# xXJSONDeruloXx/linux-fg

Hardware: AMD Instinct MI355X
Metric: interpolated frames/s, 1080p->4K RGBA8 (higher is better)
Workload: dtype f32 arithmetic on u8 RGBA (u8 in, u8 out; int8 motion vectors); 1 GPU; 1080p->2160p scale+motion(8,16)+interpolate; order=one call per stage, semantics=reference, frames_in_flight=3, content=translated (the motion stage's best case but `static`; see content_sweep), parallelism=one frame pair per GPU x1, gpu_max_hw_queues=4

## Files before the change

### linux-fg_amd/csrc/motion_strip.hip

```cpp
#include "lfg_motion_common.hpp"

#include <algorithm>
#include <vector>

namespace lfg {

constexpr int kStripPix = 64 - (kB - 1);
constexpr int kStripThreads = 1024, kStripWaves = kStripThreads / 64;
constexpr int kStripWinLane = 64 + 2 * kR;
constexpr int kStripWarm = 4;
constexpr int kStripSync = 16;
constexpr int kStripListCap = 6;
constexpr uint32_t kKeyMask = 0xFFFFF800u;
constexpr uint32_t kNearD = 3u * 2048u + 2047u;
constexpr int kStripSlots = 64 * kStripCols;

typedef const __attribute__((address_space(3))) uint32_t *strip_lds_u32;

__device__ __forceinline__ float strip_shl1(float v) {
    return __builtin_bit_cast(float, __builtin_amdgcn_mov_dpp(__builtin_bit_cast(int, v), 0x130 , 0xF, 0xF, true));
}
__device__ __forceinline__ uint32_t strip_absdiff(uint32_t a, uint32_t b) {
    uint32_t d;
    asm("v_sad_u32 %0, %1, %2, 0" : "=v"(d) : "v"(a), "v"(b));
    return d;
}
__device__ __forceinline__ void strip_record(uint32_t *cnt, uint32_t *list, uint32_t key, uint32_t floor) {
    const uint32_t at = atomicAdd(cnt, 1u) & 0x7FFFFFFFu;
    if (at < (uint32_t)kStripListCap) { list[at] = key; return; }
    for (int k = 0; k < kStripListCap; ++k) {
        const uint32_t e = list[k];
        if (key > e && key - e > kNearD) return;
    }
    for (int k = 0; k < kStripListCap; ++k) {
        const uint32_t e = list[k];
        if (e > floor && e - floor > kNearD && atomicCAS(&list[k], e, key) == e) return;
    }
    atomicOr(cnt, 0x80000000u);
}
__device__ __forceinline__ uint32_t strip_and_or(uint32_t a, uint32_t m, uint32_t r) {
    uint32_t d;
    asm("v_and_or_b32 %0, %1, %2, %3" : "=v"(d) : "v"(a), "v"(m), "s"(r));
    return d;
}
__device__ __forceinline__ float strip_sum8_lanes(float v) {
    const float t2 = v + strip_shl1(v);
    const float t4 = t2 + strip_shl1(strip_shl1(t2));
    const float t8 = t4 + strip_shl1(strip_shl1(strip_shl1(strip_shl1(t4))));
    return t8;
}

struct StripArgs {
    const uint8_t *prev, *curr;
    int prevPitch, currPitch, W, H;
    int8_t *mv; int mvPitch;
    const uint32_t *order32, *rank2scan;
    uint32_t *colBand, *rowBand;
    uint32_t *tileFlags, *flagged; int flagTilesX;
    int chunksTall, chunksWide;
};

template <bool kTall, int kOut, int kEdge, bool kRankIsScan>
__device__ __forceinline__ void strip_item(const StripArgs &a, const int L0, const int I0, const uint32_t bit, uint32_t *sWin, uint32_t *sGmin, uint32_t *sCnt, uint32_t *sList,
                                           uint16_t *sFinal, uint16_t *sHard, float (*sDist)[kB * kB], const uint16_t *sScan, uint32_t &sHardN) {
    constexpr int kIn = kOut + kB - 1;
    constexpr int kWinIn = kIn + 2 * kR;
    constexpr int kP = kWinIn | 1;
    static_assert(kOut <= kStripCols, "the LDS arrays are laid out for kStripCols pixels across the edge at most");
    const int tid = threadIdx.x, lane = tid & 63;
    const int wave = __builtin_amdgcn_readfirstlane(tid >> 6);
    const int W = a.W, H = a.H;
    const int laneSize = kTall ? H : W;
    const int wl0 = L0 - kB / 2 - kR, wi0 = I0 - kB / 2 - kR;

    constexpr int jLo = kEdge == 0 ? kB / 2 : 0, jHi = kEdge == 1 ? kIn - (kB / 2 - 1) : kIn;
    auto inImage = [](int j) constexpr { return j >= jLo && j < jHi; };
    uint32_t c[kIn], cc[kIn];
    const int gl = L0 - kB / 2 + lane;
    const bool laneIn = gl >= 0 && gl < laneSize;
    const int edgeItem = __builtin_amdgcn_readfirstlane((int)(L0 - kB / 2 < 0 || L0 - kB / 2 + 63 >= laneSize));
    {
#pragma unroll
        for (int j = jLo; j < jHi; ++j) {
            const int gi = I0 - kB / 2 + j;
            const int x = kTall ? gi : gl, y = kTall ? gl : gi;
            c[j] = *reinterpret_cast<const uint32_t *>(a.curr + (size_t)clampi(y, 0, H - 1) * (size_t)a.currPitch + (size_t)clampi(x, 0, W - 1) * 4u);
        }
    }
    for (int e = tid; e < kStripWinLane * kWinIn; e += kStripThreads) {
        const int u = kTall ? e / kWinIn : e % kStripWinLane, v = kTall ? e % kWinIn : e / kStripWinLane;
        const int x = kTall ? wi0 + v : wl0 + u, y = kTall ? wl0 + u : wi0 + v;
        const uint32_t t = *reinterpret_cast<const uint32_t *>(a.prev + (size_t)clampi(y, 0, H - 1) * (size_t)a.prevPitch + (size_t)clampi(x, 0, W - 1) * 4u);
        sWin[u * kP + v] = (x >= 0 && x < W && y >= 0 && y < H) ? t : 0u;
    }
    for (int e = tid; e < kStripSlots; e += kStripThreads) { sGmin[e] = 0xFFFFFFFFu; sCnt[e] = 0u; }
    if (tid == 0) sHardN = 0u;
#pragma unroll
    for (int j = jLo; j < jHi; ++j) {
        cc[j] = __builtin_amdgcn_udot4(c[j], c[j], 0x4B000000u, false);
        asm volatile("" : "+v"(cc[j]));
    }
    __syncthreads();

    const bool laneOk = lane < kStripPix && L0 + lane < laneSize;
    uint32_t mn[kOut];
#pragma unroll
    for (int i = 0; i < kOut; ++i) mn[i] = 0xFFFFFFFFu;
    const strip_lds_u32 winLane = (strip_lds_u32)sWin + lane * kP;
    auto leaves = [&](int px, int py, uint32_t rank) {
        const uint32_t sc = kRankIsScan ? rank : (uint32_t)sScan[min(rank, (uint32_t)kCand - 1u)];
        const int dyi = (int)((sc * 1986u) >> 16), dxi = (int)sc - 33 * dyi;
        return block_leaves_prev(px, py, dxi - kR, dyi - kR, W, H);
    };
    auto inPlateau = [&](int i, uint32_t sc) {
        const int dyi = (int)((sc * 1986u) >> 16), dxi = (int)sc - 33 * dyi, dI = (kTall ? dxi : dyi) - kR;
        const int q = I0 + i;
        return q + kB / 2 - 1 + dI < 0 || q - kB / 2 + dI >= (kTall ? W : H);
    };
    if (wave == 0) {
#pragma unroll
        for (int i = 0; i < kOut; ++i) {
            uint32_t first = (uint32_t)kCand;
            for (int r0 = 0; r0 < kCand && first == (uint32_t)kCand; r0 += 64) {
                const int r = r0 + lane;
                const unsigned long long hit = __ballot(r < kCand && inPlateau(i, kRankIsScan ? (uint32_t)r : (uint32_t)sScan[min(r, kCand - 1)]));
                if (hit != 0ull) first = (uint32_t)(r0 + __builtin_ctzll(hit));
            }
            if (lane == 0) sHard[i] = (uint16_t)first;
        }
    }
    __syncthreads();
    uint32_t rep[kOut];
#pragma unroll
    for (int i = 0; i < kOut; ++i) rep[i] = (uint32_t)__builtin_amdgcn_readfirstlane((int)sHard[i]);
    __syncthreads();
    auto adopt = [&](int i, uint32_t g) {
        if (mn[i] != g && mn[i] - g <= kNearD && !(mn[i] < 2048u && g < 2048u) && (mn[i] & 0x7FFu) % (uint32_t)kStripWaves == (uint32_t)wave) {
            const int px = kTall ? I0 + i : L0 + lane, py = kTall ? L0 + lane : I0 + i;
            const bool plateau = (mn[i] >> 11) == (g >> 11) && leaves(px, py, mn[i] & 0x7FFu) && leaves(px, py, g & 0x7FFu);
            if (!plateau) strip_record(sCnt + lane * kOut + i, sList + (lane * kOut + i) * kStripListCap, mn[i], g);
        }
        mn[i] = g;
    };

    const int lanePlus2 = ((lane + 2) & 63) * 4, lanePlus4 = ((lane + 4) & 63) * 4;
    const int nMine = (kCand - wave + kStripWaves - 1) / kStripWaves;
    for (int t = 0; t < nMine + kStripWarm; ++t) {
        if (t == kStripWarm) {
            if (laneOk) {
#pragma unroll
                for (int i = 0; i < kOut; ++i) atomicMin(&sGmin[lane * kOut + i], mn[i]);
            }
            __syncthreads();
            if (laneOk) {
#pragma unroll
                for (int i = 0; i < kOut; ++i) mn[i] = sGmin[lane * kOut + i];
            }
        }
        else if (t > kStripWarm && ((t - kStripWarm) & (kStripSync - 1)) == 0) {
            if (laneOk) {
#pragma unroll
                for (int i = 0; i < kOut; ++i) atomicMin(&sGmin[lane * kOut + i], mn[i]);
#pragma unroll
                for (int i = 0; i < kOut; ++i) adopt(i, sGmin[lane * kOut + i]);
            }
        }
        const bool recording = t >= kStripWarm;
        const int r = wave + kStripWaves * (t < nMine ? t : t - nMine);
        const uint32_t sc = kRankIsScan ? (uint32_t)r : (uint32_t)sScan[r];
        const uint32_t dyi = (sc * 1986u) >> 16, dxi = sc - 33u * dyi;
        const uint32_t off = (kTall ? dyi : dxi) * (uint32_t)kP + (kTall ? dxi : dyi);
        const strip_lds_u32 w = winLane + off;
        uint32_t p[kIn];
#pragma unroll
        for (int j = jLo; j < jHi; ++j) p[j] = w[j];
        float d[kIn];
#pragma unroll
        for (int j = jLo; j < jHi; ++j) {
            const float f1 = __builtin_bit_cast(float, __builtin_amdgcn_udot4(p[j], p[j], cc[j], false));
            const float f2 = __builtin_bit_cast(float, __builtin_amdgcn_udot4(c[j], p[j], 0x4B800000u, false));
            d[j] = __builtin_amdgcn_sqrtf((f1 - f2) + 8388608.0f);
        }
        auto sum2 = [](float x, bool xIn, float y, bool yIn) { return xIn && yIn ? x + y : xIn ? x : yIn ? y : 0.0f; };
        auto in2 = [&](int j) constexpr { return inImage(j) || inImage(j + 1); };
        auto in4 = [&](int j) constexpr { return in2(j) || in2(j + 2); };
        float a2[kIn - 1], a4[kIn - 3], h8[kOut];
#pragma unroll
        for (int j = 0; j < kIn - 1; ++j) a2[j] = sum2(inImage(j) ? d[j] : 0.0f, inImage(j), inImage(j + 1) ? d[j + 1] : 0.0f, inImage(j + 1));
#pragma unroll
        for (int j = 0; j < kIn - 3; ++j) a4[j] = sum2(a2[j], in2(j), a2[j + 2], in2(j + 2));
#pragma unroll
        for (int i = 0; i < kOut; ++i) h8[i] = sum2(a4[i], in4(i), a4[i + 4], in4(i + 4));
        if (edgeItem) {
            asm volatile("; lanes outside the image (strip)");
#pragma unroll
            for (int i = 0; i < kOut; ++i) h8[i] = laneIn ? h8[i] : 0.0f;
        }
        float t2[kOut], t4[kOut], sum[kOut];
#pragma unroll
        for (int i = 0; i < kOut; ++i) t2[i] = h8[i] + strip_shl1(h8[i]);
#pragma unroll
        for (int i = 0; i < kOut; ++i) t4[i] = __builtin_bit_cast(float, __builtin_amdgcn_ds_bpermute(lanePlus2, __builtin_bit_cast(int, t2[i])));
#pragma unroll
        for (int i = 0; i < kOut; ++i) t4[i] = t2[i] + t4[i];
#pragma unroll
        for (int i = 0; i < kOut; ++i) sum[i] = __builtin_bit_cast(float, __builtin_amdgcn_ds_bpermute(lanePlus4, __builtin_bit_cast(int, t4[i])));
        uint32_t key[kOut], nearMin = 0xFFFFFFFFu;
#pragma unroll
        for (int i = 0; i < kOut; ++i) {
            const float s = t4[i] + sum[i];
            key[i] = strip_and_or(__builtin_bit_cast(uint32_t, s), kKeyMask, (uint32_t)r) | ((inPlateau(i, sc) && (uint32_t)r != rep[i]) ? 0xFFFFFFFFu : 0u);
            nearMin = min(nearMin, strip_absdiff(key[i], mn[i]));
        }
        nearMin = laneOk ? nearMin : 0xFFFFFFFFu;
        if (recording && __builtin_amdgcn_readfirstlane((int)(__ballot(nearMin <= kNearD) != 0ull))) {
            asm volatile("; near event (strip)");
#pragma unroll
            for (int i = 0; i < kOut; ++i) {
                const bool near = laneOk && strip_absdiff(key[i], mn[i]) <= kNearD;
                if (__builtin_amdgcn_readfirstlane((int)(__ballot(near) != 0ull))) {
                    if (near) {
                        const int px = kTall ? I0 + i : L0 + lane, py = kTall ? L0 + lane : I0 + i;
                        const uint32_t holder = mn[i];
                        bool skip = (key[i] < 2048u && holder < 2048u) || key[i] == holder;
                        if (!skip && (key[i] >> 11) == (holder >> 11)) skip = leaves(px, py, (uint32_t)r) && leaves(px, py, holder & 0x7FFu);
                        if (key[i] < holder && (holder & 0x7FFu) % (uint32_t)kStripWaves != (uint32_t)wave) skip = true;
                        if (!skip) strip_record(sCnt + lane * kOut + i, sList + (lane * kOut + i) * kStripListCap, max(key[i], holder), min(key[i], holder));
                    }
                }
            }
        }
#pragma unroll
        for (int i = 0; i < kOut; ++i) mn[i] = min(mn[i], key[i]);
    }

    if (laneOk) {
#pragma unroll
        for (int i = 0; i < kOut; ++i) atomicMin(&sGmin[lane * kOut + i], mn[i]);
    }
    __syncthreads();
    if (laneOk) {
#pragma unroll
        for (int i = 0; i < kOut; ++i) adopt(i, sGmin[lane * kOut + i]);
    }
    __syncthreads();
    for (int e = tid; e < kStripSlots; e += kStripThreads) {
        const int l = e / kOut, i = e - l * kOut;
        if (l >= kStripPix || L0 + l >= laneSize) continue;
        const uint32_t g = sGmin[e], n = sCnt[e];
        sFinal[e] = (uint16_t)(g & 0x7FFu);
        if (g < 2048u || n == 0u) continue;
        uint32_t live = 0u;
        for (uint32_t k = 0; k < min(n & 0x7FFFFFFFu, (uint32_t)kStripListCap); ++k) {
            const uint32_t key = sList[e * kStripListCap + k];
            live += (key >= g && key - g <= kNearD && key != g) ? 1u : 0u;
        }
        if ((n >> 31) != 0u) {
            const int px = kTall ? I0 + i : L0 + l, py = kTall ? L0 + l : I0 + i;
            if (atomicExch(&a.tileFlags[(py / kTH) * a.flagTilesX + px / kTW], 1u) == 0u) {
                const uint32_t slot = atomicAdd(a.flagged, 1u);
                if (slot < (uint32_t)kShareBelow) a.flagged[1 + slot] = (uint32_t)((py / kTH) * a.flagTilesX + px / kTW);
            }
            continue;
        }
        if (live == 0u) continue;
        sHard[atomicAdd(&sHardN, 1u)] = (uint16_t)e;
    }
    __syncthreads();
    const uint32_t hardN = sHardN;
    for (uint32_t hI = (uint32_t)wave; hI < hardN; hI += (uint32_t)kStripWaves) {
        const int e = (int)sHard[hI];
        const int l = e / kOut, i = e - l * kOut;
        const int qx = kTall ? I0 + i : L0 + l, qy = kTall ? L0 + l : I0 + i;
        const uint32_t g = sGmin[e];
        const uint32_t n = min(sCnt[e] & 0x7FFFFFFFu, (uint32_t)kStripListCap);
        uint32_t mine = 0xFFFFFFFFu;
        if (lane == 0) mine = g;
        else if ((uint32_t)lane <= n) { const uint32_t k = sList[e * kStripListCap + lane - 1]; mine = (k >= g && k - g <= kNearD) ? k : 0xFFFFFFFFu; }
        const int cx = qx - kB / 2 + (lane & 7), cy = qy - kB / 2 + (lane >> 3);
        const bool posIn = cx >= 0 && cx < W && cy >= 0 && cy < H;
        const uint32_t ctex = posIn ? *reinterpret_cast<const uint32_t *>(a.curr + (size_t)cy * (size_t)a.currPitch + (size_t)cx * 4u) : 0u;
        const float cf[4] = {unorm8_to_float(byte0(ctex)), unorm8_to_float(byte1(ctex)), unorm8_to_float(byte2(ctex)), unorm8_to_float(byte3(ctex))};
        float bestV = __builtin_inff();
        uint32_t bestR = 0xFFFFFFFFu, done = 0xFFFFFFFFu;
        unsigned long long todo = __ballot(mine != 0xFFFFFFFFu);
        while (todo != 0ull) {
            const int b = __builtin_ctzll(todo);
            todo &= todo - 1ull;
            const uint32_t rank = (uint32_t)__builtin_amdgcn_readlane((int)mine, b) & 0x7FFu;
            if (rank == done) continue;
            done = rank;
            const int scan = (int)a.rank2scan[rank];
            const int dy = scan / kSide - kR, dx = scan % kSide - kR;
            const int sx = cx + dx, sy = cy + dy;
            uint32_t ptex = 0u;
            if (posIn && sx >= 0 && sy >= 0 && sx < W && sy < H)
                ptex = *reinterpret_cast<const uint32_t *>(a.prev + (size_t)sy * (size_t)a.prevPitch + (size_t)sx * 4u);
            const f32x4 pp = {unorm8_to_float(byte0(ptex)), unorm8_to_float(byte1(ptex)), unorm8_to_float(byte2(ptex)), unorm8_to_float(byte3(ptex))};
            sDist[wave][lane] = posIn ? dist4<true>(cf, pp) : 0.0f;
            wave_lds_sync();
            float v = 0.0f;
#pragma unroll
            for (int k = 0; k < kB * kB; ++k) v += sDist[wave][k];
            wave_lds_sync();
            uint32_t rr = rank;
            if (block_leaves_prev(qx, qy, dx, dy, W, H)) {
                for (uint32_t r0 = 0; r0 < rank; r0 += 64u) {
                    const uint32_t t = r0 + (uint32_t)lane;
                    const unsigned long long hit = __ballot(t < rank && leaves(qx, qy, t));
                    if (hit != 0ull) { rr = r0 + (uint32_t)__builtin_ctzll(hit); break; }
                }
            }
            if (v < bestV || (v == bestV && rr < bestR)) { bestV = v; bestR = rr; }
        }
        if (lane == 0) sFinal[e] = (uint16_t)bestR;
    }
    __syncthreads();
    for (int e = tid; e < kStripSlots; e += kStripThreads) {
        const int l = e / kOut, i = e - l * kOut;
        if (l >= kStripPix || L0 + l >= laneSize) continue;
        const int px = kTall ? I0 + i : L0 + l, py = kTall ? L0 + l : I0 + i;
        const int scan = (int)a.rank2scan[sFinal[e]];
        const int dyi = scan / kSide, dxi = scan - dyi * kSide;
        *reinterpret_cast<uint16_t *>(a.mv + (size_t)py * (size_t)a.mvPitch + (size_t)px * 2u) = mv_word(dxi - kR, dyi - kR);
    }
    if (tid < kStripPix && L0 + tid < laneSize) atomicOr(&(kTall ? a.colBand : a.rowBand)[L0 + tid], bit);
}

template <bool kRankIsScan>
__global__ __launch_bounds__(kStripThreads) void motion_strip_kernel(StripArgs a) {
    constexpr int kPmax = (kStripCols + kB - 1 + 2 * kR) | 1;
    __shared__ uint32_t sWin[kStripWinLane * kPmax];
    __shared__ uint32_t sGmin[kStripSlots], sCnt[kStripSlots];
    __shared__ uint32_t sList[kStripSlots * kStripListCap];
    __shared__ uint16_t sFinal[kStripSlots], sHard[kStripSlots];
    __shared__ float sDist[kStripWaves][kB * kB];
    __shared__ uint16_t sScan[kRankIsScan ? 2 : kCand + 1];
    __shared__ uint32_t sHardN;
    const int item = (int)blockIdx.x;
    const int side = item < 2 * a.chunksTall ? item / a.chunksTall : 2 + (item - 2 * a.chunksTall) / a.chunksWide;
    const int chunk = item < 2 * a.chunksTall ? item % a.chunksTall : (item - 2 * a.chunksTall) % a.chunksWide;
    const uint32_t top = a.order32[0];
    const int dx = (int)((top >> 16) / (uint32_t)kWinH) - kR, dy = (int)((top >> 16) % (uint32_t)kWinH) - kR;
    const bool active = side == 0 ? dx < 0 : side == 1 ? dx > 0 : side == 2 ? dy < 0 : dy > 0;
    if (!active) return;
    if (!kRankIsScan) {
        for (int i = threadIdx.x; i < kCand; i += kStripThreads) sScan[i] = (uint16_t)a.rank2scan[i];
        __syncthreads();
    }
    const int L0 = chunk * kStripPix;
#define LFG_STRIP_ITEM(tall, across, edge, i0) strip_item<tall, across, edge, kRankIsScan>(a, L0, i0, 1u << (side & 1), sWin, sGmin, sCnt, sList, sFinal, sHard, sDist, sScan, sHardN)
    if (side == 0) LFG_STRIP_ITEM(true, kStripCols, 0, 0);
    else if (side == 1) LFG_STRIP_ITEM(true, kStripCols, 1, a.W - kStripCols);
    else if (side == 2) LFG_STRIP_ITEM(false, kStripRows, 0, 0);
    else LFG_STRIP_ITEM(false, kStripRows, 1, a.H - kStripRows);
#undef LFG_STRIP_ITEM
}

bool strip_frames_ok(const lfg_frame &prev, const lfg_frame &curr, const lfg_frame &mv) {
    return curr.width >= 256u && curr.height >= 256u && (mv.pitch & 1u) == 0u && ((uintptr_t)mv.data & 1u) == 0u;
}

hipError_t launch_motion_strip(hipStream_t s, const lfg_frame &prev, const lfg_frame &curr, const lfg_frame &mv, const uint32_t *order32,
                               const uint32_t *rank2scan, bool rankIsScan, uint32_t *colBand, uint32_t *rowBand,
                               uint32_t *tileFlags, uint32_t *flagged, int flagTilesX, int ldsPad) {
    StripArgs a;
    a.prev = (const uint8_t *)prev.data; a.curr = (const uint8_t *)curr.data;
    a.prevPitch = (int)prev.pitch; a.currPitch = (int)curr.pitch; a.W = (int)curr.width; a.H = (int)curr.height;
    a.mv = (int8_t *)mv.data; a.mvPitch = (int)mv.pitch;
    a.order32 = order32; a.rank2scan = rank2scan; a.colBand = colBand; a.rowBand = rowBand;
    a.tileFlags = tileFlags; a.flagged = flagged; a.flagTilesX = flagTilesX;
    a.chunksTall = (a.H + kStripPix - 1) / kStripPix; a.chunksWide = (a.W + kStripPix - 1) / kStripPix;
    const int items = 2 * a.chunksTall + 2 * a.chunksWide;
    if (rankIsScan) hipLaunchKernelGGL(motion_strip_kernel<true>, dim3((unsigned)items), dim3(kStripThreads), (size_t)ldsPad, s, a);
    else hipLaunchKernelGGL(motion_strip_kernel<false>, dim3((unsigned)items), dim3(kStripThreads), (size_t)ldsPad, s, a);
    return hipGetLastError();
}

}
```

Before: 3928 frames/s.

## Precompute plateau masks per displacement and batch bpermutes in strip motion kernel

Each displacement index now gets a per-band-pixel plateau bitmask, built once into LDS, so the per-candidate plateau test becomes a uniform LDS lookup with a fast path when no pixel is in the plateau. The lane-rotation reductions issue all ds_bpermute ops in one asm block with a single wait, and the scan index is made wave-uniform via readfirstlane. Near-event detection reuses the precomputed absolute differences and masks out invalid lanes with a ballot. Inline asm with hard waits limits how the compiler can schedule around these instructions, and the extra LDS array adds a little shared-memory pressure.

New measurement: 3928 frames/s, median of 3. About the same (+0.0%).

```diff
diff --git a/linux-fg_amd/csrc/motion_strip.hip b/linux-fg_amd/csrc/motion_strip.hip
--- a/linux-fg_amd/csrc/motion_strip.hip
+++ b/linux-fg_amd/csrc/motion_strip.hip
@@ -43,6 +43,25 @@
     asm("v_and_or_b32 %0, %1, %2, %3" : "=v"(d) : "v"(a), "v"(m), "s"(r));
     return d;
 }
+template <int kOut>
+__device__ __forceinline__ void strip_permute_all(float (&out)[kOut], const int addr, const float (&v)[kOut]) {
+    static_assert(kOut == 8 || kOut == 12, "one statement per band width");
+    if constexpr (kOut == 8) {
+        asm("ds_bpermute_b32 %0, %8, %9\n\tds_bpermute_b32 %1, %8, %10\n\tds_bpermute_b32 %2, %8, %11\n\tds_bpermute_b32 %3, %8, %12\n\t"
+            "ds_bpermute_b32 %4, %8, %13\n\tds_bpermute_b32 %5, %8, %14\n\tds_bpermute_b32 %6, %8, %15\n\tds_bpermute_b32 %7, %8, %16\n\t"
+            "s_waitcnt lgkmcnt(0)"
+            : "=&v"(out[0]), "=&v"(out[1]), "=&v"(out[2]), "=&v"(out[3]), "=&v"(out[4]), "=&v"(out[5]), "=&v"(out[6]), "=&v"(out[7])
+            : "v"(addr), "v"(v[0]), "v"(v[1]), "v"(v[2]), "v"(v[3]), "v"(v[4]), "v"(v[5]), "v"(v[6]), "v"(v[7]));
+    } else {
+        asm("ds_bpermute_b32 %0, %12, %13\n\tds_bpermute_b32 %1, %12, %14\n\tds_bpermute_b32 %2, %12, %15\n\tds_bpermute_b32 %3, %12, %16\n\t"
+            "ds_bpermute_b32 %4, %12, %17\n\tds_bpermute_b32 %5, %12, %18\n\tds_bpermute_b32 %6, %12, %19\n\tds_bpermute_b32 %7, %12, %20\n\t"
+            "ds_bpermute_b32 %8, %12, %21\n\tds_bpermute_b32 %9, %12, %22\n\tds_bpermute_b32 %10, %12, %23\n\tds_bpermute_b32 %11, %12, %24\n\t"
+            "s_waitcnt lgkmcnt(0)"
+            : "=&v"(out[0]), "=&v"(out[1]), "=&v"(out[2]), "=&v"(out[3]), "=&v"(out[4]), "=&v"(out[5]), "=&v"(out[6]), "=&v"(out[7]),
+              "=&v"(out[8]), "=&v"(out[9]), "=&v"(out[10]), "=&v"(out[11])
+            : "v"(addr), "v"(v[0]), "v"(v[1]), "v"(v[2]), "v"(v[3]), "v"(v[4]), "v"(v[5]), "v"(v[6]), "v"(v[7]), "v"(v[8]), "v"(v[9]), "v"(v[10]), "v"(v[11]));
+    }
+}
 __device__ __forceinline__ float strip_sum8_lanes(float v) {
     const float t2 = v + strip_shl1(v);
     const float t4 = t2 + strip_shl1(strip_shl1(t2));
@@ -62,7 +81,7 @@
 
 template <bool kTall, int kOut, int kEdge, bool kRankIsScan>
 __device__ __forceinline__ void strip_item(const StripArgs &a, const int L0, const int I0, const uint32_t bit, uint32_t *sWin, uint32_t *sGmin, uint32_t *sCnt, uint32_t *sList,
-                                           uint16_t *sFinal, uint16_t *sHard, float (*sDist)[kB * kB], const uint16_t *sScan, uint32_t &sHardN) {
+                                           uint16_t *sFinal, uint16_t *sHard, float (*sDist)[kB * kB], const uint16_t *sScan, uint32_t *sPlat, uint32_t &sHardN) {
     constexpr int kIn = kOut + kB - 1;
     constexpr int kWinIn = kIn + 2 * kR;
     constexpr int kP = kWinIn | 1;
@@ -112,11 +131,21 @@
         const int dyi = (int)((sc * 1986u) >> 16), dxi = (int)sc - 33 * dyi;
         return block_leaves_prev(px, py, dxi - kR, dyi - kR, W, H);
     };
-    auto inPlateau = [&](int i, uint32_t sc) {
-        const int dyi = (int)((sc * 1986u) >> 16), dxi = (int)sc - 33 * dyi, dI = (kTall ? dxi : dyi) - kR;
-        const int q = I0 + i;
+    auto inPlateauAt = [&](int i, int dIdx) {
+        const int q = I0 + i, dI = dIdx - kR;
         return q + kB / 2 - 1 + dI < 0 || q - kB / 2 + dI >= (kTall ? W : H);
     };
+    auto inPlateau = [&](int i, uint32_t sc) {
+        const int dyi = (int)((sc * 1986u) >> 16), dxi = (int)sc - 33 * dyi;
+        return inPlateauAt(i, kTall ? dxi : dyi);
+    };
+    if (tid >= kStripThreads - kSide) {
+        const int dIdx = tid - (kStripThreads - kSide);
+        uint32_t m = 0u;
+#pragma unroll
+        for (int i = 0; i < kOut; ++i) m |= inPlateauAt(i, dIdx) ? 1u << i : 0u;
+        sPlat[dIdx] = m;
+    }
     if (wave == 0) {
 #pragma unroll
         for (int i = 0; i < kOut; ++i) {
@@ -130,9 +159,7 @@
         }
     }
     __syncthreads();
-    uint32_t rep[kOut];
-#pragma unroll
-    for (int i = 0; i < kOut; ++i) rep[i] = (uint32_t)__builtin_amdgcn_readfirstlane((int)sHard[i]);
+    const uint32_t repLane = lane < kOut ? (uint32_t)sHard[lane] : 0xFFFFFFFFu;
     __syncthreads();
     auto adopt = [&](int i, uint32_t g) {
         if (mn[i] != g && mn[i] - g <= kNearD && !(mn[i] < 2048u && g < 2048u) && (mn[i] & 0x7FFu) % (uint32_t)kStripWaves == (uint32_t)wave) {
@@ -143,6 +170,7 @@
         mn[i] = g;
     };
 
+    const unsigned long long okLanes = __ballot(laneOk);
     const int lanePlus2 = ((lane + 2) & 63) * 4, lanePlus4 = ((lane + 4) & 63) * 4;
     const int nMine = (kCand - wave + kStripWaves - 1) / kStripWaves;
     for (int t = 0; t < nMine + kStripWarm; ++t) {
@@ -167,10 +195,11 @@
         }
         const bool recording = t >= kStripWarm;
         const int r = wave + kStripWaves * (t < nMine ? t : t - nMine);
-        const uint32_t sc = kRankIsScan ? (uint32_t)r : (uint32_t)sScan[r];
+        const uint32_t sc = kRankIsScan ? (uint32_t)r : (uint32_t)__builtin_amdgcn_readfirstlane((int)sScan[r]);
         const uint32_t dyi = (sc * 1986u) >> 16, dxi = sc - 33u * dyi;
         const uint32_t off = (kTall ? dyi : dxi) * (uint32_t)kP + (kTall ? dxi : dyi);
         const strip_lds_u32 w = winLane + off;
+        const uint32_t plat = sPlat[kTall ? dxi : dyi];
         uint32_t p[kIn];
 #pragma unroll
         for (int j = jLo; j < jHi; ++j) p[j] = w[j];
@@ -196,36 +225,41 @@
 #pragma unroll
             for (int i = 0; i < kOut; ++i) h8[i] = laneIn ? h8[i] : 0.0f;
         }
-        float t2[kOut], t4[kOut], sum[kOut];
+        float t2[kOut], far2[kOut], t4[kOut], far4[kOut];
 #pragma unroll
         for (int i = 0; i < kOut; ++i) t2[i] = h8[i] + strip_shl1(h8[i]);
-#pragma unroll
-        for (int i = 0; i < kOut; ++i) t4[i] = __builtin_bit_cast(float, __builtin_amdgcn_ds_bpermute(lanePlus2, __builtin_bit_cast(int, t2[i])));
-#pragma unroll
-        for (int i = 0; i < kOut; ++i) t4[i] = t2[i] + t4[i];
-#pragma unroll
-        for (int i = 0; i < kOut; ++i) sum[i] = __builtin_bit_cast(float, __builtin_amdgcn_ds_bpermute(lanePlus4, __builtin_bit_cast(int, t4[i])));
+        strip_permute_all<kOut>(far2, lanePlus2, t2);
+#pragma unroll
+        for (int i = 0; i < kOut; ++i) t4[i] = t2[i] + far2[i];
+        strip_permute_all<kOut>(far4, lanePlus4, t4);
+        const uint32_t never = (uint32_t)__builtin_amdgcn_readfirstlane((int)plat) & ~(uint32_t)__ballot(repLane == (uint32_t)r);
         uint32_t key[kOut], nearMin = 0xFFFFFFFFu;
-#pragma unroll
-        for (int i = 0; i < kOut; ++i) {
-            const float s = t4[i] + sum[i];
-            key[i] = strip_and_or(__builtin_bit_cast(uint32_t, s), kKeyMask, (uint32_t)r) | ((inPlateau(i, sc) && (uint32_t)r != rep[i]) ? 0xFFFFFFFFu : 0u);
-            nearMin = min(nearMin, strip_absdiff(key[i], mn[i]));
-        }
-        nearMin = laneOk ? nearMin : 0xFFFFFFFFu;
-        if (recording && __builtin_amdgcn_readfirstlane((int)(__ballot(nearMin <= kNearD) != 0ull))) {
-            asm volatile("; near event (strip)");
+        if (never == 0u) {
+#pragma unroll
+            for (int i = 0; i < kOut; ++i) key[i] = strip_and_or(__builtin_bit_cast(uint32_t, t4[i] + far4[i]), kKeyMask, (uint32_t)r);
+        } else {
+#pragma unroll
+            for (int i = 0; i < kOut; ++i)
+                key[i] = strip_and_or(__builtin_bit_cast(uint32_t, t4[i] + far4[i]), kKeyMask, (uint32_t)r | (0u - ((never >> i) & 1u)));
+        }
+        uint32_t apart[kOut];
+#pragma unroll
+        for (int i = 0; i < kOut; ++i) { apart[i] = strip_absdiff(key[i], mn[i]); nearMin = min(nearMin, apart[i]); }
+        if (recording && (__ballot(nearMin <= kNearD) & okLanes) != 0ull) {
+            asm volatile("; near event (strip)" : "+v"(apart[0]));
 #pragma unroll
             for (int i = 0; i < kOut; ++i) {
-                const bool near = laneOk && strip_absdiff(key[i], mn[i]) <= kNearD;
-                if (__builtin_amdgcn_readfirstlane((int)(__ballot(near) != 0ull))) {
-                    if (near) {
-                        const int px = kTall ? I0 + i : L0 + lane, py = kTall ? L0 + lane : I0 + i;
+                const bool near = apart[i] <= kNearD;
+                if ((__ballot(near) & okLanes) != 0ull) {
+                    if (near && laneOk) {
+                        int me = lane;
+                        asm volatile("" : "+v"(me));
+                        const int px = kTall ? I0 + i : L0 + me, py = kTall ? L0 + me : I0 + i;
                         const uint32_t holder = mn[i];
                         bool skip = (key[i] < 2048u && holder < 2048u) || key[i] == holder;
                         if (!skip && (key[i] >> 11) == (holder >> 11)) skip = leaves(px, py, (uint32_t)r) && leaves(px, py, holder & 0x7FFu);
                         if (key[i] < holder && (holder & 0x7FFu) % (uint32_t)kStripWaves != (uint32_t)wave) skip = true;
-                        if (!skip) strip_record(sCnt + lane * kOut + i, sList + (lane * kOut + i) * kStripListCap, max(key[i], holder), min(key[i], holder));
+                        if (!skip) strip_record(sCnt + me * kOut + i, sList + (me * kOut + i) * kStripListCap, max(key[i], holder), min(key[i], holder));
                     }
                 }
             }
@@ -336,6 +370,7 @@
     __shared__ uint16_t sFinal[kStripSlots], sHard[kStripSlots];
     __shared__ float sDist[kStripWaves][kB * kB];
     __shared__ uint16_t sScan[kRankIsScan ? 2 : kCand + 1];
+    __shared__ uint32_t sPlat[kSide];
     __shared__ uint32_t sHardN;
     const int item = (int)blockIdx.x;
     const int side = item < 2 * a.chunksTall ? item / a.chunksTall : 2 + (item - 2 * a.chunksTall) / a.chunksWide;
@@ -349,7 +384,7 @@
         __syncthreads();
     }
     const int L0 = chunk * kStripPix;
-#define LFG_STRIP_ITEM(tall, across, edge, i0) strip_item<tall, across, edge, kRankIsScan>(a, L0, i0, 1u << (side & 1), sWin, sGmin, sCnt, sList, sFinal, sHard, sDist, sScan, sHardN)
+#define LFG_STRIP_ITEM(tall, across, edge, i0) strip_item<tall, across, edge, kRankIsScan>(a, L0, i0, 1u << (side & 1), sWin, sGmin, sCnt, sList, sFinal, sHard, sDist, sScan, sPlat, sHardN)
     if (side == 0) LFG_STRIP_ITEM(true, kStripCols, 0, 0);
     else if (side == 1) LFG_STRIP_ITEM(true, kStripCols, 1, a.W - kStripCols);
     else if (side == 2) LFG_STRIP_ITEM(false, kStripRows, 0, 0);
```
